# LemonATsu/DANBO-pytorch

Hardware: AMD Instinct MI355X
Metric: ray-samples/sec at 512x512x64 samples (higher is better)
Workload: dtype f32 (fp16x2-split MFMA products, fp32 accumulate); 1 GPU; H36M danbo_base network, 512x512 rays x (48 coarse + 16 importance) samples, 1 pose / 1 camera per rank, cylinder near/far, exact in-volume culling; rays=262144, samples_per_ray=64, parallelism=rays-dp1

## Files before the change

### danbo-pytorch_amd/core/_hip.py

```python
import ctypes
import os
import re
from ctypes import c_char_p, c_float, c_int, c_void_p
from types import SimpleNamespace

import torch

_HERE = os.path.dirname(os.path.abspath(__file__))
LIB_PATH = os.environ.get("DANBO_HIP_LIB") or os.path.join(os.path.dirname(_HERE), "libdanbo_hip.so")

P = c_void_p
I = c_int
F = c_float


class HeaderError(ValueError):
    """include/danbo_hip.h left the subset of C that parse_header reads"""


_SCALARS = {"int": c_int, "long": ctypes.c_long, "long long": ctypes.c_longlong, "size_t": ctypes.c_size_t, "float": c_float,
            **{f"{u}int{n}_t": getattr(ctypes, f"c_{u}int{n}") for u in ("", "u") for n in (8, 16, 32, 64)}}
_TAIL = r"((?:\*\s*(?:const\b\s*)?)*)(\w+)\s*(?:\[\s*(\w*)\s*\])?$"
_DECL = re.compile(r"(?:const\s+)?(long\s+long|\w+)\b\s*" + _TAIL)
_MORE = re.compile(_TAIL)
# ... 137 lines not shown
    return functions, structs, constants


def _header_path():
    env = os.environ.get("DANBO_HIP_HEADER")
    tried = [env] if env else [os.path.join(os.path.dirname(LIB_PATH), "danbo_hip.h"),
                               os.path.join(os.path.dirname(os.path.dirname(_HERE)), "include", "danbo_hip.h")]
    for p in tried:
        if os.path.exists(p):
            return p
    raise RuntimeError("danbo_hip.h not found (the ctypes binding is derived from it): tried " + ", ".join(tried)
                       + "; set DANBO_HIP_HEADER or put the header beside the library")


HEADER_PATH = _header_path()
with open(HEADER_PATH) as _f:
    _functions, _structs, _constants = parse_header(_f.read())
SIGNATURES = {name: argtypes for name, (_, argtypes) in _functions.items()}
RESTYPES = {name: restype for name, (restype, _) in _functions.items()}
STRUCTS = {name: type(name, (ctypes.Structure,), {"_fields_": fields, "__doc__": f"struct {name} of include/danbo_hip.h"})
           for name, fields in _structs.items()}
globals().update(STRUCTS)
C = SimpleNamespace(**_constants)
MAX_ROW_SPANS = C.DANBO_MAX_ROW_SPANS
ANERF_MAX_D = C.DANBO_ANERF_MAX_D

TRAIN_TENSORS = (
    ["graph_net.layers.0.lin.weight", "graph_net.layers.0.adj_w", "graph_net.layers.0.bias", "graph_net.layers.1.lin.weight",
     "graph_net.layers.1.adj_w", "graph_net.layers.1.bias", "graph_net.layers.2.weight", "graph_net.layers.2.bias",
     "graph_net.layers.3.weight", "graph_net.layers.3.bias", "graph_net.axis_scale",
     "prob_linears.layers.0.lin.weight", "prob_linears.layers.0.adj_w", "prob_linears.layers.0.bias", "prob_linears.layers.1.weight",
     "prob_linears.layers.1.bias", "prob_linears.layers.2.weight", "prob_linears.layers.2.bias"]
    + [f"pts_linears.{i}.weight" for i in range(8)] + [f"pts_linears.{i}.bias" for i in range(8)]
    + ["alpha_linear.weight", "alpha_linear.bias", "feature_linear.weight", "feature_linear.bias", "views_linears.0.weight",
       "views_linears.0.bias", "rgb_linear.weight", "rgb_linear.bias", "framecodes.codes.weight"])
N_TRAIN_TENSORS = C.DANBO_T_COUNT
_anchors = {"graph_net.axis_scale": C.DANBO_T_AXIS_SCALE, "prob_linears.layers.0.lin.weight": C.DANBO_T_A_W0,
            "pts_linears.0.weight": C.DANBO_T_PTS_W0, "pts_linears.0.bias": C.DANBO_T_PTS_B0, "alpha_linear.weight": C.DANBO_T_ALPHA_W,
            "framecodes.codes.weight": C.DANBO_T_CODES}
if len(TRAIN_TENSORS) != N_TRAIN_TENSORS or any(TRAIN_TENSORS.index(k) != i for k, i in _anchors.items()):
    raise HeaderError(f"TRAIN_TENSORS does not line up with enum DanboTrainTensor of {HEADER_PATH}")

_lib = None


def lib():
    global _lib
    if _lib is None:
        if not os.path.exists(LIB_PATH):
            raise RuntimeError(
                f"{LIB_PATH} not found: build it with `make -C danbo-pytorch_amd/csrc` "
                "(or __graft_entry__.build()).  There is no CPU / PyTorch fallback.")
        l = ctypes.CDLL(LIB_PATH)
        for name, argtypes in SIGNATURES.items():
            fn = getattr(l, name)
            fn.argtypes = argtypes
            fn.restype = RESTYPES[name]
        if l.danbo_abi_version() != C.DANBO_ABI_VERSION:
            raise RuntimeError(f"{LIB_PATH} has ABI version {l.danbo_abi_version()}, {HEADER_PATH} declares {C.DANBO_ABI_VERSION}: "
                               "the library is stale, rebuild it with `make -C danbo-pytorch_amd/csrc`")
        _lib = l
    return _lib


def ptr(t):
    return None if t is None else c_void_p(t.data_ptr())


def stream():
    return c_void_p(torch.cuda.current_stream().cuda_stream)


class HipError(RuntimeError):
    pass


def check(code, name):
    if code != 0:
        raise HipError(f"{name} failed with code {code}" + (" (invalid argument)" if code == C.DANBO_EINVAL else ""))

# ... 4 lines not shown
```

### danbo-pytorch_amd/core/hip_ops.py

```python
import ctypes

import torch

from . import _hip
from ._hip import call as _call, ptr as _p, stream as _stream

J = _hip.C.DANBO_J
VOL = _hip.C.DANBO_VOL
FEAT = _hip.C.DANBO_FEAT
RAY_FLAT_VMAX = _hip.C.DANBO_RAY_FLAT_VMAX
H_STRIDE = _hip.C.DANBO_H_STRIDE
MLP_PACKED_FLOATS = _hip.C.DANBO_MLP_PACKED_FLOATS
ASSIGN16_PACKED_BYTES = _hip.C.DANBO_ASSIGN16_PACKED_BYTES
MLP16_PACKED_BYTES = _hip.C.DANBO_MLP16_PACKED_BYTES
ANERF_ENC_FLOATS = _hip.C.DANBO_ANERF_ENC_FLOATS
LINEAR16_ENC_K = _hip.C.DANBO_LINEAR16_ENC_K
TRUNK_PACKED_BYTES = _hip.C.DANBO_TRUNK_PACKED_BYTES
TRUNK_PE_WIDTH = _hip.C.DANBO_TRUNK_PE_WIDTH
VIEW_W = 128


def _f32(t, name):
    if t is None:
        return None
# ... 70 lines not shown
        self.S = self.z.shape[1] if self.z is not None else self.pts.shape[1]
        self.M = self.R * self.S
        self.device = self.rays_o.device
        self.ray_mask = ray_mask if self.z is not None else None

    def head(self):
        return (_p(self.rays_o), _p(self.rays_d), _p(self.z), _p(self.pts), self.R, self.S, self.G,
                _p(self.skts), _p(self.align), _p(self.axis_scale))


def bone_cull(geo, compact=True, cnt=None):
    bits = torch.empty(geo.M, device=geo.device, dtype=torch.int32)
    lst = None
    if compact:
        lst = torch.empty(geo.M, device=geo.device, dtype=torch.int32)
        if cnt is None:
            cnt = torch.zeros(1, device=geo.device, dtype=torch.int32)
        assert cnt.dtype == torch.int32 and cnt.numel() == 1 and cnt.is_contiguous()
    else:
        cnt = None
    rm = tuple(geo.ray_mask) if geo.ray_mask is not None else (None, None, None)
    flat = rm[3] if len(rm) > 3 else None
    _call("danbo_bone_cull", *geo.head(), _p(rm[0]), _p(rm[1]), _p(rm[2]), _p(flat), _p(bits), _p(lst), _p(cnt), _stream())
    return bits, lst, cnt


def ray_bone_mask(rays_o, rays_d, skts, align, axis_scale, t_lo, t_hi, want_flat=False):
    rays_o, rays_d, skts = _f32(rays_o, "rays_o"), _f32(rays_d, "rays_d"), _f32(skts, "skts")
    t_lo, t_hi = _f32(t_lo, "t_lo").reshape(-1), _f32(t_hi, "t_hi").reshape(-1)
    R, G = rays_o.shape[0], skts.shape[0]
    assert t_lo.shape[0] == R and t_hi.shape[0] == R
    mask = torch.empty(R, device=rays_o.device, dtype=torch.int32)
    flat = torch.empty(R, device=rays_o.device, dtype=torch.int32) if want_flat else None
    _call("danbo_ray_bone_mask", _p(rays_o), _p(rays_d), _p(t_lo), _p(t_hi), R, G, _p(skts), _p(_f32(align, "align")),
          _p(_f32(axis_scale, "axis_scale")), _p(mask), _p(flat), _stream())
    return (mask, t_lo, t_hi, flat) if want_flat else (mask, t_lo, t_hi)


def group_rows(bits, lst, cnt):
    _call("danbo_group_rows", _p(bits), _p(lst), _p(cnt), lst.shape[0], _stream())
    return lst


def bone_gather(geo, volumes, lst=None, cnt=None, n=None):
    n = geo.M if n is None else n
    out = torch.empty(n, J, FEAT, device=geo.device, dtype=torch.float32)
# ... 618 lines not shown
```

### danbo-pytorch_amd/core/render_engine.py

```python
import ctypes

import torch

from . import _hip
from . import hip_ops as ops


class RenderEngine:
    fuse_resample = False

    def _key(self):
        return tuple((k, v.data_ptr(), v._version) for k, v in sorted(self.p.items()))

    def _sampling(self, N_samples, N_importance):
        cfg = self.cfg
        return (N_samples or cfg["N_samples"], N_importance or cfg["N_importance"], cfg["density_scale"],
                ops.density_act(cfg.get("density_act")))

    @staticmethod
    def frame_result(out, out0):
        return dict(rgb_map=out["rgb_map"], disp_map=out["disp_map"], acc_map=out["acc_map"], alpha=out["alpha"],
                    T_i=out["weights"], rgb0=out0["rgb_map"], disp0=out0["disp_map"], acc0=out0["acc_map"],
                    alpha0=out0["alpha"])

# ... 20 lines not shown
        ret = self.frame_result(out, out0)
        if keep:
            ret.update(near=near, far=far, z_coarse=z, raw_coarse=raw, weights_coarse=out0["weights"], z_fine=z_fine,
                       z_sorted=z_all, sorted_idxs=order, raw_fine=raw_f, **ex, **ex_f)
        return ret


class DanboEngine(RenderEngine):
    fuse_resample = True

    def __init__(self, cfg, params, align, buffers=None, mlp_mode="f16split"):
        self.cfg = cfg
        self.p = params
        self.align = align.float().contiguous()
        self._packed_key = None
        self.packed = self.wrt = self.empty_consts = None
        self.mean_code = None
        self.profile = None
        self.skip_flat_rays = True
        self.mlp_form = 32
        assert mlp_mode in ("f16split", "fp32")
        self.mlp_mode = mlp_mode
        self.group_rows = False

    def refresh(self):
        key = self._key()
        if key == self._packed_key and getattr(self, "_built_mode", None) == (self.mlp_mode, self.mlp_form):
            return
        p = self.p
        dev = p["alpha_linear.weight"].device
        q = self._equalized(p) if self.mlp_mode == "f16split" else p
        self.pts_w = [q[f"pts_linears.{i}.weight"] for i in range(8)]
        self.pts_b = [q[f"pts_linears.{i}.bias"].contiguous() for i in range(8)]
        self.packed, self.wrt = ops.mlp_pack(self.pts_w, q["feature_linear.weight"], q["views_linears.0.weight"])
        self.packed16, self.views_b16 = ops.mlp16_pack(self.pts_w, q["feature_linear.weight"],
                                                       q["feature_linear.bias"], q["views_linears.0.weight"],
                                                       q["views_linears.0.bias"], form=self.mlp_form)
        self.alpha_w = q["alpha_linear.weight"].reshape(-1).contiguous()
        self.alpha_b = q["alpha_linear.bias"].contiguous()
        self.feature_b = q["feature_linear.bias"].contiguous()
        self.views_b = q["views_linears.0.bias"].contiguous()
        self.rgb_w = q["rgb_linear.weight"].contiguous()
        self.rgb_b = q["rgb_linear.bias"].contiguous()
        self.view_scale = q.get("_view_scale", torch.ones((), device=dev))
        g = "graph_net.layers."
        self.gw = dict(
# ... 87 lines not shown
    def _mlp(self, h, S, cview, raw, lst=None, cnt=None, n=None, aux=False):
        if self.mlp_mode == "f16split":
            return ops.pe_mlp16(h, S, self.packed16, self.pts_b, self.alpha_w, self.alpha_b, cview,
                                self.rgb_w, self.rgb_b, raw, lst, cnt, n, aux, form=self.mlp_form)
        return ops.pe_mlp(h, S, self.packed, self.pts_b, self.alpha_w, self.alpha_b, self.feature_b, cview,
                          self.rgb_w, self.rgb_b, raw, lst, cnt, n, aux)

    def volumes(self, bones):
        self.refresh()
        return ops.pose_volumes(bones, self.gw, self.cfg["multires_graph"])

    def view_constants(self, rays_d, skts, cam_idx, ray_list=None, ray_count=None):
        self.refresh()
        cfg = self.cfg
        ray_mode = {"world": 0, "root_local": 1}[cfg["ray_tr_type"]]
        normalise = 1 if cfg["view_type"] == "relray" else 0
        return ops.view_consts(rays_d, skts, ray_mode, normalise, cfg["multires_views"], self.framecodes,
                               self.mean_code, cam_idx, self.wrt,
                               self.views_b16 if self.mlp_mode == "f16split" else self.views_b, self.rgb_w,
                               self.rgb_b, self.empty_consts, {16: 1, 32: 2}[self.mlp_form] if self.mlp_mode == "f16split" else 0,
                               self.code_table, ray_list, ray_count)

    def forward_samples(self, rays_o, rays_d, skts, bones, cam_idx=None, z=None, pts=None, dense=False,
                        want_confd=False, volumes=None, view=None, fill=True, ray_mask=None, count=None):
        self.refresh()
        geo = ops.Geometry(rays_o, rays_d, skts, self.align, self.axis_scale, z=z, pts=pts, ray_mask=ray_mask)
        vols = self.volumes(bones) if volumes is None else volumes
        cview, raw_empty = self.view_constants(geo.rays_d, geo.skts, cam_idx) if view is None else view
        S = geo.S
        bits, lst, cnt = ops.bone_cull(geo, compact=not dense, cnt=count)
        if lst is not None and self.mlp_mode == "f16split" and self.group_rows:
            ops.group_rows(bits, lst, cnt)
        if self.mlp_mode == "f16split":
            h, confd = ops.gather_assign_blend16(geo, vols, bits, self.aw, self.assign16, lst, cnt, geo.M, want_confd)
        else:
            h, confd = ops.gather_assign_blend(geo, vols, bits, self.aw, lst, cnt, geo.M, want_confd)
        raw = ops.fill_raw(raw_empty, S) if fill or dense else torch.empty(geo.R, S, 4, device=raw_empty.device)
        if self.profile is not None:
            e0, e1 = torch.cuda.Event(enable_timing=True), torch.cuda.Event(enable_timing=True)
            e0.record()
        self._mlp(h, S, cview, raw, lst, cnt, geo.M)
        if self.profile is not None:
            e1.record()
            self.profile.setdefault("k_pe_mlp", []).append((e0, e1, cnt if cnt is not None else geo.M))
        extras = dict(valid_bits=bits, list=lst, count=cnt, confd_rows=confd, h_rows=h, volumes=vols)
        return raw, extras

    def density(self, pts, skts, bones, netchunk=1024 * 64):
        self.refresh()
        M = pts.shape[0]
        out = torch.empty(M, 1, device=pts.device, dtype=torch.float32)
        vols = self.volumes(bones)
        for a in range(0, M, netchunk):
# ... 50 lines not shown
        m.density_scale, m.use_volume_near_far = float(cfg["density_scale"]), int(bool(cfg["use_volume_near_far"]))
        m.flat_rays_ok = int(self.flat_rays_ok and self.skip_flat_rays)
        r = _hip.DanboRays(rays_o=rays_o.data_ptr(), rays_d=rays_d.data_ptr(), skts=skts.data_ptr(), bones=bones.data_ptr(),
                           cyls=cyls.data_ptr(), cam_idx=None if cam is None else cam.data_ptr(), near_in=None, far_in=None,
                           R=R, G=G, chunk=int(chunk))
        shapes = dict(rgb_map=(R, 3), disp_map=(R,), acc_map=(R,), alpha=(R, S + Sf), weights=(R, S + Sf), rgb0=(R, 3),
                      disp0=(R,), acc0=(R,), alpha0=(R, S))
        out = {k: torch.empty(v, device=dev, dtype=torch.float32) for k, v in shapes.items()}
        o = _hip.DanboFrameOut(**{k: v.data_ptr() for k, v in out.items()})
        nbytes = _hip.lib().danbo_render_frame_workspace(R, G, S, Sf, int(chunk), m.graph_width)
        ws = torch.empty(nbytes, device=dev, dtype=torch.uint8)
        ops._call("danbo_render_frame_act", ctypes.byref(m), ctypes.byref(r), S, Sf, ctypes.byref(o), _hip.ptr(ws), nbytes,
                  *ops._act_args(act), ops._stream())
        out["T_i"] = out.pop("weights")
        return out

    def near_far(self, rays_o, rays_d, cyls, skts, near0=0.0, far0=1.0, chunk=4096):
        self.refresh()
        near, far = ops.near_far_cylinder(rays_o, rays_d, cyls, near0, far0, chunk)
        if self.cfg["use_volume_near_far"]:
            ops.near_far_boxes(rays_o, rays_d, skts, self.align, self.axis_scale, near, far)
        return near, far

    def render(self, rays_o, rays_d, skts, bones, cyls, cam_idx=None, N_samples=None, N_importance=None,
               chunk=4096, near_far=None, dense=False, keep=False):
        S, Sf, B, act = self._sampling(N_samples, N_importance)
        self.refresh()
        fused = S <= 64 and Sf <= 64
        lazy = not dense and not keep
        flat_mode = (lazy and (fused or (S <= 256 and Sf <= 64)) and self.skip_flat_rays and self.flat_rays_ok
                     and act[0] == "relu")
        near, far = self.near_far(rays_o, rays_d, cyls, skts, 0.0, 1.0, chunk) if near_far is None else near_far
        z = ops.coarse_samples(near, far, S)
        ray_mask = None if dense else ops.ray_bone_mask(rays_o, rays_d, skts, self.align, self.axis_scale, near, far,
                                                        want_flat=flat_mode)
        counts = torch.zeros(3, device=rays_o.device, dtype=torch.int32)
        flat = None
        vols = self.volumes(bones)
        if flat_mode:
            flat = ops.flat_rays(ray_mask[1], ray_mask[3], S, Sf, want_weights=not fused, cnt=counts[2:3])
            view = self.view_constants(rays_d, skts, cam_idx, flat["ray_list"], flat["ray_count"])
        else:
            view = self.view_constants(rays_d, skts, cam_idx)
        if ray_mask is not None:
            ray_mask = ray_mask[:3]
        raw, ex = self.forward_samples(rays_o, rays_d, skts, bones, cam_idx, z=z, dense=dense, volumes=vols, view=view,
                                       fill=not lazy, ray_mask=ray_mask, count=counts[0:1])
        if fused:
            out0, z_all, z_fine, order = ops.composite_importance(
                raw, z, rays_d, Sf, B, bits=ex["valid_bits"] if lazy else None, raw_empty=view[1] if lazy else None,
                want_weights=keep, flat=flat, act=act)
        else:
            out0 = ops.composite(raw, z, rays_d, B, bits=ex["valid_bits"] if lazy else None, raw_empty=view[1] if lazy else None,
                                 flat=flat, act=act)
            z_all, z_fine, order = ops.importance_samples(z, out0["weights"], Sf, flat=flat)
        raw_f, ex_f = self.forward_samples(rays_o, rays_d, skts, bones, cam_idx, z=z_fine, dense=dense,
                                           volumes=vols, view=view, fill=not lazy,
                                           ray_mask=ray_mask, count=counts[1:2])
        out = ops.composite_merged(raw, raw_f, order, z_all, rays_d, B, bits_a=ex["valid_bits"] if lazy else None,
                                   bits_b=ex_f["valid_bits"] if lazy else None, raw_empty=view[1] if lazy else None,
                                   want_raw=keep, flat=flat, act=act)
        ret = self.frame_result(out, out0)
        if keep:
            ret.update(near=near, far=far, z_coarse=z, raw_coarse=raw, weights_coarse=out0["weights"], z_fine=z_fine,
                       z_sorted=z_all, sorted_idxs=order, raw_fine=raw_f, raw_sorted=out.get("raw_sorted"),
                       count_coarse=ex["count"], count_fine=ex_f["count"], valid_bits=ex["valid_bits"])
        return ret

    def _network_pass(self, rays_o, rays_d, skts, bones, cam_idx, z, bounds, dense, lazy, tag):
        mask = None if dense else ops.ray_bone_mask(rays_o, rays_d, skts, self.align, self.axis_scale, *bounds)
        view = self.view_constants(rays_d, skts, cam_idx)
        raw, ex = self.forward_samples(rays_o, rays_d, skts, bones, cam_idx, z=z, dense=dense, volumes=self.volumes(bones), view=view,
                                       fill=not lazy, ray_mask=mask)
        bits, empty = (ex["valid_bits"], view[1]) if lazy else (None, None)
        return raw, bits, empty, {"count_" + tag: ex["count"], "valid_bits" + ("_fine" if tag == "fine" else ""): ex["valid_bits"]}
```

### danbo-pytorch_amd/csrc/common.hpp

```cpp
#pragma once
#include <hip/hip_runtime.h>
#include <stdint.h>
#include <algorithm>
#include <atomic>
#include "../../include/danbo_hip.h"
#include "sample_math.hpp"

#define DANBO_CHECK_ARG(cond) do { if (!(cond)) return DANBO_EINVAL; } while (0)
#define DANBO_CHECK_DENSITY_ACT(act, shift) \
    DANBO_CHECK_ARG(((act) == DANBO_DENSITY_RELU || (act) == DANBO_DENSITY_SOFTPLUS) && (shift) - (shift) == 0.f)
#define DANBO_LAUNCH_RET() do { hipError_t e_ = hipGetLastError(); return e_ == hipSuccess ? 0 : (int)e_; } while (0)

#define DANBO_ENSURE_LDS(func, bytes)                                                                              \
    do {                                                                                                           \
        static std::atomic<unsigned long long> done_{0};                                                           \
        int dev_ = 0;                                                                                              \
        if (hipGetDevice(&dev_) != hipSuccess) return (int)hipGetLastError();                                      \
        const unsigned long long bit_ = 1ull << (dev_ & 63);                                                       \
        if (!(done_.load(std::memory_order_acquire) & bit_)) {                                                     \
            const hipError_t e_ = hipFuncSetAttribute(reinterpret_cast<const void*>(func),                         \
                                                      hipFuncAttributeMaxDynamicSharedMemorySize, (int)(bytes));   \
            if (e_ != hipSuccess) return (int)e_;                                                                  \
            done_.fetch_or(bit_, std::memory_order_release);                                                       \
        }                                                                                                          \
    } while (0)

#if defined(__HIP_DEVICE_COMPILE__)
#define DANBO_NO_PK_F32 __attribute__((target("no-packed-fp32-ops")))
// ... 160 lines not shown
```

### danbo-pytorch_amd/csrc/k_frame.hip

```cpp
#include "common.hpp"

using namespace danbo;

namespace {
struct Carver {
    char* base;
    size_t used, cap;
    template <class T>
    T* take(size_t n) {
        used = (used + 255) & ~(size_t)255;
        T* p = base ? reinterpret_cast<T*>(base + used) : nullptr;
        used += n * sizeof(T);
        return p;
    }
};

struct FrameBuffers {
    float *near, *far, *cyl_scratch, *z, *vol_scratch, *volumes, *cview, *raw_empty, *h, *raw_a, *raw_b, *z_fine, *z_sorted, *weights0;
    uint32_t *bits_a, *bits_b, *ray_mask, *ray_flat;
    int32_t *list, *count, *order, *ray_list;
};

FrameBuffers carve(Carver& c, int R, int G, int S, int Sf, int chunk, int Wg) {
    FrameBuffers b;
// ... 31 lines not shown
    carve(c, R, G, S, Sf, chunk, graph_width);
    return c.used + 256;
}

#define DANBO_TRY(call) do { const int rc_ = (call); if (rc_ != 0) return rc_; } while (0)

static int render_frame_impl(const DanboModel* m, const DanboRays* r, int S, int Sf, const DanboFrameOut* o, void* workspace,
                             size_t workspace_bytes, int act, float shift, void* stream) {
    DANBO_CHECK_ARG(m && r && o && workspace && S >= 3 && S <= 256 && Sf >= 1 && Sf <= 64);
    DANBO_CHECK_ARG(r->R >= 1 && r->G >= 1 && r->R % r->G == 0 && r->chunk >= 1);
    DANBO_CHECK_ARG(r->rays_o && r->rays_d && r->skts && r->bones && r->cyls);
    DANBO_CHECK_ARG(o->rgb_map && o->disp_map && o->acc_map && o->alpha && o->weights && o->rgb0 && o->disp0 && o->acc0 && o->alpha0);
    const int R = r->R, G = r->G;
    const bool flat_rays = m->flat_rays_ok != 0 && act == DANBO_DENSITY_RELU;
    DANBO_CHECK_ARG(workspace_bytes >= danbo_render_frame_workspace(R, G, S, Sf, r->chunk, m->graph_width));
    Carver c{reinterpret_cast<char*>(((uintptr_t)workspace + 255) & ~(uintptr_t)255), 0, workspace_bytes};
    const FrameBuffers b = carve(c, R, G, S, Sf, r->chunk, m->graph_width);
    hipStream_t st = (hipStream_t)stream;

    DANBO_TRY(danbo_near_far_cylinder(r->rays_o, r->rays_d, r->cyls, R, G, 0.f, 1.f, r->near_in, r->far_in, r->chunk, b.cyl_scratch,
                                      b.near, b.far, stream));
    if (m->use_volume_near_far)
        DANBO_TRY(danbo_near_far_boxes(r->rays_o, r->rays_d, r->skts, m->align, m->axis_scale, R, G, b.near, b.far, stream));
    DANBO_TRY(danbo_coarse_samples(b.near, b.far, R, S, nullptr, b.z, stream));
    DANBO_TRY(danbo_ray_bone_mask(r->rays_o, r->rays_d, b.near, b.far, R, G, r->skts, m->align, m->axis_scale, b.ray_mask,
                                  flat_rays ? b.ray_flat : nullptr, stream));
    DANBO_TRY(danbo_pose_volumes_fwd(r->bones, G, m->L_graph, m->graph_width, m->g_w0, m->g_adjw0, m->g_b0, m->g_w1, m->g_adjw1, m->g_b1,
                                     m->g_w2, m->g_b2, m->g_w3, m->g_b3, b.vol_scratch, b.volumes, stream));
    zero_words(b.count, 4, nullptr, 0, st);
    auto view_consts = [&](const int32_t* ray_list, const int32_t* ray_count) -> int {
        return danbo_view_consts(r->rays_d, r->skts, R, G, m->ray_mode, m->normalise, m->L_view, m->framecodes, m->n_codes, m->code_size,
                                 m->mean_code, r->cam_idx, m->views_w_ray_t, m->views_b_eff, m->rgb_w, m->rgb_b, m->empty_consts, 2,
                                 m->code_table, ray_list, ray_count, b.cview, b.raw_empty, stream);
    };
    const int32_t *ray_list = nullptr, *ray_count = nullptr;
    if (flat_rays) {
        DANBO_TRY(danbo_flat_rays(b.near, b.ray_flat, R, S, Sf, o->rgb0, o->disp0, o->acc0, b.weights0, o->alpha0, b.z_fine, o->rgb_map,
                                  o->disp_map, o->acc_map, o->weights, o->alpha, b.ray_list, b.count + 3, 3, stream));
        ray_list = b.ray_list;
        ray_count = b.count + 3;
    }
    DANBO_TRY(view_consts(ray_list, ray_count));
    auto cull = [&](const float* zz, int s, uint32_t* bits, int32_t* count) -> int {
        DANBO_TRY(danbo_bone_cull(r->rays_o, r->rays_d, zz, nullptr, R, s, G, r->skts, m->align, m->axis_scale, b.ray_mask, b.near, b.far,
                                  nullptr, bits, b.list, count, stream));
        return 0;
    };
    auto network = [&](const float* zz, int s, uint32_t* bits, int32_t* count, float* raw) -> int {
        DANBO_TRY(danbo_gather_assign_blend16_fwd(r->rays_o, r->rays_d, zz, nullptr, R, s, G, r->skts, m->align, m->axis_scale, b.volumes,
                                                  bits, b.list, count, R * s, m->assign16, m->a_b0, m->a_b1, m->a_w2, m->a_b2, b.h,
                                                  nullptr, reinterpret_cast<uint32_t*>(b.count + 2), stream));
        return danbo_pe_mlp32_fwd(b.h, b.list, count, R * s, s, m->mlp16, m->pts_b, m->alpha_w, m->alpha_b, b.cview, m->rgb_w,
                                  m->rgb_b, raw, nullptr, stream);
    };
    DANBO_TRY(cull(b.z, S, b.bits_a, b.count));
    DANBO_TRY(network(b.z, S, b.bits_a, b.count, b.raw_a));
    if (S <= 64) {
        DANBO_TRY(danbo_composite_importance_pdf_fwd_act(b.raw_a, b.raw_empty, b.bits_a, b.z, r->rays_d, R, S, Sf, m->density_scale, nullptr,
                                                         nullptr, 0, o->rgb0, o->disp0, o->acc0, nullptr, o->alpha0, b.z_fine, b.z_sorted,
                                                         b.order, ray_list, ray_count, act, shift, stream));
    } else {
        DANBO_TRY(danbo_composite_rays_fwd_act(b.raw_a, b.raw_empty, b.bits_a, b.z, r->rays_d, R, S, m->density_scale, nullptr, o->rgb0,
                                               o->disp0, o->acc0, b.weights0, o->alpha0, ray_list, ray_count, act, shift, stream));
        DANBO_TRY(danbo_importance_samples_rays(b.z, b.weights0, R, S, Sf, nullptr, b.z_fine, b.z_sorted, b.order, ray_list, ray_count,
                                                stream));
    }
// ... 18 lines not shown
```

### danbo-pytorch_amd/csrc/k_sample.hip

```cpp
#include "common.hpp"

namespace danbo {

__global__ __launch_bounds__(256) DANBO_NO_PK_F32 void k_cylinder_pass1(const float* __restrict__ rays_o,
                                                        const float* __restrict__ rays_d,
                                                        const float* __restrict__ cyl, int R, int G,
                                                        float near0, float far0,
                                                        const float* __restrict__ near_in,
                                                        const float* __restrict__ far_in, int chunk,
                                                        double* __restrict__ acc,
                                                        float* __restrict__ near_out,
                                                        float* __restrict__ far_out) {
    const int rays_per_pose = R / G;
    for (int r0 = blockIdx.x * blockDim.x; r0 < R; r0 += gridDim.x * blockDim.x) {
        const int r = r0 + threadIdx.x;
        const bool act = r < R;
        const int rc = act ? r : R - 1;
        const int g = min(rc / rays_per_pose, G - 1);
        float o[3] = {rays_o[3 * rc], rays_o[3 * rc + 1], rays_o[3 * rc + 2]};
        float d[3] = {rays_d[3 * rc], rays_d[3 * rc + 1], rays_d[3 * rc + 2]};
        float c[3] = {cyl[5 * g], cyl[5 * g + 1], cyl[5 * g + 2]};
        float nr, fr;
        const bool hit = cylinder_bounds(o, d, c, near_in ? near_in[rc] : near0, far_in ? far_in[rc] : far0, &nr, &fr) && act;
        if (act) {
// ... 490 lines not shown
    if (list != nullptr) {
        __shared__ int s_cnt[CULL_SPT * (CULL_BLOCK / 64)];
        __shared__ int s_base;
        const int wave = threadIdx.x >> 6;
        unsigned long long ball[CULL_SPT];
#pragma unroll
        for (int it = 0; it < CULL_SPT; ++it) {
            ball[it] = __ballot(bits4[it] != 0);
            if (lane == 0) s_cnt[it * (CULL_BLOCK / 64) + wave] = __popcll(ball[it]);
        }
        __syncthreads();
        if (threadIdx.x == 0) {
            int run = 0;
            for (int i = 0; i < CULL_SPT * (CULL_BLOCK / 64); ++i) { const int c = s_cnt[i]; s_cnt[i] = run; run += c; }
            s_base = run > 0 ? atomicAdd(count, run) : 0;
        }
        __syncthreads();
#pragma unroll
        for (int it = 0; it < CULL_SPT; ++it) {
            if (bits4[it] != 0) {
                const long m = base + it * CULL_BLOCK + threadIdx.x;
                list[s_base + s_cnt[it * (CULL_BLOCK / 64) + wave] + __popcll(ball[it] & ((1ull << lane) - 1ull))] = (int32_t)m;
            }
        }
    }
}

constexpr int GATHER_TS = 16;
constexpr int GATHER_BLOCK = GATHER_TS * J;

__global__ __launch_bounds__(GATHER_BLOCK) void k_bone_gather(const float* __restrict__ rays_o,
                                                              const float* __restrict__ rays_d,
                                                              const float* __restrict__ z,
                                                              const float* __restrict__ pts, int R, int S, int G,
                                                              const float* __restrict__ skts,
                                                              const float* __restrict__ align,
                                                              const float* __restrict__ axis_scale,
                                                              const float* __restrict__ volumes,
                                                              const int32_t* __restrict__ list,
                                                              const int32_t* __restrict__ count, int n_cap,
                                                              float* __restrict__ part_feat) {
    __shared__ __attribute__((aligned(16))) float s_vol[J * VOL];
    __shared__ __attribute__((aligned(16))) float s_out[GATHER_TS * J * FEAT];
    __shared__ __attribute__((aligned(16))) float s_skt[J * 16];
    __shared__ __attribute__((aligned(16))) float s_align[J * 16];
    __shared__ float s_scale[J * 4];
// ... 607 lines not shown

extern "C" int danbo_bone_cull(const float* rays_o, const float* rays_d, const float* z, const float* pts, int R, int S, int G,
                                const float* skts, const float* align, const float* axis_scale, const uint32_t* ray_mask,
                                const float* t_lo, const float* t_hi, uint32_t* ray_flat, uint32_t* valid_bits, int32_t* list,
                                int32_t* count, void* stream) {
    DANBO_CHECK_ARG(R > 0 && S > 0 && G > 0 && R % G == 0);
    DANBO_CHECK_ARG((list == nullptr) == (count == nullptr));
    DANBO_CHECK_ARG((z == nullptr) != (pts == nullptr));
    DANBO_CHECK_ARG(ray_mask == nullptr || (z != nullptr && t_lo != nullptr && t_hi != nullptr));
    DANBO_CHECK_ARG(ray_flat == nullptr || ray_mask != nullptr);
    const long M = (long)R * S;
    const long spp = (long)(R / G) * S;
    const int per_block = CULL_BLOCK * CULL_SPT;
    long np = per_block / spp + 2;
    if (np > G) np = G;
    const size_t lds = sizeof(float) * (J * 16 + J * 4 + np * J * 16);
    DANBO_CHECK_ARG(lds <= 64 * 1024);
    const int grid = ceil_div(M, per_block);
    hipLaunchKernelGGL(k_bone_cull, dim3(grid), dim3(CULL_BLOCK), lds, (hipStream_t)stream, rays_o, rays_d, z, pts, R, S,
                       G, skts, align, axis_scale, (int)np, ray_mask, t_lo, t_hi, ray_flat, valid_bits, list, count);
    DANBO_LAUNCH_RET();
}

extern "C" int danbo_ray_bone_mask(const float* rays_o, const float* rays_d, const float* t_lo, const float* t_hi, int R, int G,
                                    const float* skts, const float* align, const float* axis_scale, uint32_t* ray_mask,
                                    uint32_t* ray_flat, void* stream) {
    DANBO_CHECK_ARG(rays_o && rays_d && t_lo && t_hi && skts && align && axis_scale && ray_mask);
    DANBO_CHECK_ARG(R > 0 && G > 0 && R % G == 0);
    const long np = 256 / (R / G) + 2 < G ? 256 / (R / G) + 2 : G;
    const bool in_lds = np <= 8;
    const size_t lds = sizeof(float) * (J * 16 + J * 4 + (in_lds ? np * J * 16 : 0));
    if (in_lds)
        hipLaunchKernelGGL(k_ray_bone_mask<true>, dim3(ceil_div(R, 256)), dim3(256), lds, (hipStream_t)stream, rays_o, rays_d, t_lo, t_hi,
                           skts, align, axis_scale, R, G, ray_mask, ray_flat);
    else
        hipLaunchKernelGGL(k_ray_bone_mask<false>, dim3(ceil_div(R, 256)), dim3(256), lds, (hipStream_t)stream, rays_o, rays_d, t_lo,
                           t_hi, skts, align, axis_scale, R, G, ray_mask, ray_flat);
    DANBO_LAUNCH_RET();
}

extern "C" int danbo_bone_gather_fwd(const float* rays_o, const float* rays_d, const float* z, const float* pts, int R, int S, int G,
                                      const float* skts, const float* align, const float* axis_scale,
                                      const float* volumes, const int32_t* list, const int32_t* count, int n,
                                      float* part_feat, void* stream) {
    DANBO_CHECK_ARG(R > 0 && S > 0 && G > 0 && R % G == 0 && n >= 0);
    DANBO_CHECK_ARG((z == nullptr) != (pts == nullptr));
// ... 227 lines not shown
```

Measured before the change: 4.146 billion ray-samples/s.

## Cull samples only over listed non-flat rays, fusing coarse depth generation

Adds a bone-cull kernel that walks the compacted ray list from flat_rays instead of every sample of every ray. Each block takes a window of listed rays, computes coarse depths on the fly and writes them out, which replaces the separate coarse_samples pass. It then tests bone volumes and compacts the surviving sample rows with an LDS histogram that can optionally group rows by bone pair. Rays left out of the list never get coarse depths or valid bits written, so downstream code must not read them. The per-block ray grouping also adds LDS scan overhead.

```diff
diff --git a/danbo-pytorch_amd/core/_hip.py b/danbo-pytorch_amd/core/_hip.py
--- a/danbo-pytorch_amd/core/_hip.py
+++ b/danbo-pytorch_amd/core/_hip.py
@@ -183,6 +183,20 @@
            for name, fields in _structs.items()}
 globals().update(STRUCTS)
 C = SimpleNamespace(**_constants)
+COMPANION_HEADERS = ("danbo_hip_rays.h",)
+COMPANION_SIGNATURES, COMPANION_RESTYPES, _companion_constants = {}, {}, {}
+for _name in COMPANION_HEADERS:
+    _path = os.path.join(os.path.dirname(HEADER_PATH), _name)
+    if not os.path.exists(_path):
+        raise RuntimeError(f"{_path} not found: it belongs beside {HEADER_PATH}")
+    with open(_path) as _f:
+        _fns, _sts, _cons = parse_header(_f.read())
+    if _sts or set(_fns) & (set(SIGNATURES) | set(COMPANION_SIGNATURES)) or set(_cons) & (set(_constants) | set(_companion_constants)):
+        raise HeaderError(f"{_path}: a companion header declares entry points and constants only, each once")
+    _companion_constants.update(_cons)
+    COMPANION_SIGNATURES.update({name: argtypes for name, (_, argtypes) in _fns.items()})
+    COMPANION_RESTYPES.update({name: restype for name, (restype, _) in _fns.items()})
+COMPANION_C = SimpleNamespace(**_companion_constants)
 MAX_ROW_SPANS = C.DANBO_MAX_ROW_SPANS
 ANERF_MAX_D = C.DANBO_ANERF_MAX_D
 
@@ -213,10 +227,10 @@
                 f"{LIB_PATH} not found: build it with `make -C danbo-pytorch_amd/csrc` "
                 "(or __graft_entry__.build()).  There is no CPU / PyTorch fallback.")
         l = ctypes.CDLL(LIB_PATH)
-        for name, argtypes in SIGNATURES.items():
+        for name, argtypes in {**SIGNATURES, **COMPANION_SIGNATURES}.items():
             fn = getattr(l, name)
             fn.argtypes = argtypes
-            fn.restype = RESTYPES[name]
+            fn.restype = RESTYPES[name] if name in RESTYPES else COMPANION_RESTYPES[name]
         if l.danbo_abi_version() != C.DANBO_ABI_VERSION:
             raise RuntimeError(f"{LIB_PATH} has ABI version {l.danbo_abi_version()}, {HEADER_PATH} declares {C.DANBO_ABI_VERSION}: "
                                "the library is stale, rebuild it with `make -C danbo-pytorch_amd/csrc`")
diff --git a/danbo-pytorch_amd/core/hip_ops.py b/danbo-pytorch_amd/core/hip_ops.py
--- a/danbo-pytorch_amd/core/hip_ops.py
+++ b/danbo-pytorch_amd/core/hip_ops.py
@@ -116,6 +116,46 @@
     rm = tuple(geo.ray_mask) if geo.ray_mask is not None else (None, None, None)
     flat = rm[3] if len(rm) > 3 else None
     _call("danbo_bone_cull", *geo.head(), _p(rm[0]), _p(rm[1]), _p(rm[2]), _p(flat), _p(bits), _p(lst), _p(cnt), _stream())
+    return bits, lst, cnt
+
+
+CULL_RAYS_MAX_WINDOW = _hip.COMPANION_C.DANBO_CULL_RAYS_MAX_WINDOW
+CULL_RAYS_MAX_RPW = _hip.COMPANION_C.DANBO_CULL_RAYS_MAX_RPW
+
+
+def cull_rays_check(R, S, ray_mask, ray_list, ray_count, near_far=None, rpw=0):
+    if ray_mask is None or len(ray_mask) < 3 or any(t is None for t in ray_mask[:3]):
+        raise ValueError("bone_cull_rays needs ray_bone_mask()'s (mask, t_lo, t_hi) of the rays")
+    if any(t.numel() != R for t in ray_mask[:3]) or ray_mask[0].dtype != torch.int32:
+        raise ValueError("ray mask, t_lo, t_hi: one entry per ray, the mask int32")
+    if ray_list is None or ray_count is None:
+        raise ValueError("bone_cull_rays walks a ray list: pass flat_rays()'s ray_list and ray_count (no list: bone_cull)")
+    if ray_list.dtype != torch.int32 or ray_list.numel() < R or not ray_list.is_contiguous():
+        raise ValueError("ray_list: contiguous int32 with room for every ray")
+    if ray_count.dtype != torch.int32 or ray_count.numel() != 1:
+        raise ValueError("ray_count: one int32")
+    if near_far is not None and any(t.dtype != torch.float32 or t.numel() != R or not t.is_contiguous() for t in near_far):
+        raise ValueError("near_far: two contiguous float32 [R]")
+    rpw = int(rpw)
+    if rpw < 0 or rpw > CULL_RAYS_MAX_RPW or max(rpw, 1) * S > CULL_RAYS_MAX_WINDOW:
+        raise ValueError(f"rays per window {rpw} x {S} samples: at most {CULL_RAYS_MAX_RPW} rays and {CULL_RAYS_MAX_WINDOW} samples")
+    return rpw
+
+
+def bone_cull_rays(geo, ray_list, ray_count, cnt=None, near_far=None, by_bone=True, rpw=0):
+    if geo.z is None:
+        raise ValueError("bone_cull_rays works on depths along rays (Geometry(z=...)), not on points")
+    rpw = cull_rays_check(geo.R, geo.S, geo.ray_mask, ray_list, ray_count, near_far, rpw)
+    bits = torch.empty(geo.M, device=geo.device, dtype=torch.int32)
+    lst = torch.empty(geo.M, device=geo.device, dtype=torch.int32)
+    if cnt is None:
+        cnt = torch.zeros(1, device=geo.device, dtype=torch.int32)
+    assert cnt.dtype == torch.int32 and cnt.numel() == 1 and cnt.is_contiguous()
+    rm = geo.ray_mask
+    nf = (None, None) if near_far is None else near_far
+    _call("danbo_bone_cull_rays", _p(geo.rays_o), _p(geo.rays_d), _p(None if near_far is not None else geo.z), _p(nf[0]), _p(nf[1]),
+          _p(geo.z if near_far is not None else None), geo.R, geo.S, geo.G, _p(geo.skts), _p(geo.align), _p(geo.axis_scale),
+          _p(rm[0]), _p(rm[1]), _p(rm[2]), _p(ray_list), _p(ray_count), rpw, int(bool(by_bone)), _p(bits), _p(lst), _p(cnt), _stream())
     return bits, lst, cnt
 
 
diff --git a/danbo-pytorch_amd/core/render_engine.py b/danbo-pytorch_amd/core/render_engine.py
--- a/danbo-pytorch_amd/core/render_engine.py
+++ b/danbo-pytorch_amd/core/render_engine.py
@@ -66,6 +66,8 @@
         assert mlp_mode in ("f16split", "fp32")
         self.mlp_mode = mlp_mode
         self.group_rows = False
+        self.cull_listed_rays = True
+        self.cull_rows_by_bone = False
 
     def refresh(self):
         key = self._key()
@@ -199,13 +201,17 @@
                                self.code_table, ray_list, ray_count)
 
     def forward_samples(self, rays_o, rays_d, skts, bones, cam_idx=None, z=None, pts=None, dense=False,
-                        want_confd=False, volumes=None, view=None, fill=True, ray_mask=None, count=None):
+                        want_confd=False, volumes=None, view=None, fill=True, ray_mask=None, count=None, rays=None, near_far=None):
         self.refresh()
         geo = ops.Geometry(rays_o, rays_d, skts, self.align, self.axis_scale, z=z, pts=pts, ray_mask=ray_mask)
         vols = self.volumes(bones) if volumes is None else volumes
         cview, raw_empty = self.view_constants(geo.rays_d, geo.skts, cam_idx) if view is None else view
         S = geo.S
-        bits, lst, cnt = ops.bone_cull(geo, compact=not dense, cnt=count)
+        if rays is not None:
+            assert not dense
+            bits, lst, cnt = ops.bone_cull_rays(geo, rays[0], rays[1], cnt=count, near_far=near_far, by_bone=self.cull_rows_by_bone)
+        else:
+            bits, lst, cnt = ops.bone_cull(geo, compact=not dense, cnt=count)
         if lst is not None and self.mlp_mode == "f16split" and self.group_rows:
             ops.group_rows(bits, lst, cnt)
         if self.mlp_mode == "f16split":
@@ -302,6 +308,9 @@
             ops.near_far_boxes(rays_o, rays_d, skts, self.align, self.axis_scale, near, far)
         return near, far
 
+    def list_cull(self, flat_mode):
+        return bool(flat_mode) and bool(self.cull_listed_rays)
+
     def render(self, rays_o, rays_d, skts, bones, cyls, cam_idx=None, N_samples=None, N_importance=None,
                chunk=4096, near_far=None, dense=False, keep=False):
         S, Sf, B, act = self._sampling(N_samples, N_importance)
@@ -311,21 +320,24 @@
         flat_mode = (lazy and (fused or (S <= 256 and Sf <= 64)) and self.skip_flat_rays and self.flat_rays_ok
                      and act[0] == "relu")
         near, far = self.near_far(rays_o, rays_d, cyls, skts, 0.0, 1.0, chunk) if near_far is None else near_far
-        z = ops.coarse_samples(near, far, S)
         ray_mask = None if dense else ops.ray_bone_mask(rays_o, rays_d, skts, self.align, self.axis_scale, near, far,
                                                         want_flat=flat_mode)
         counts = torch.zeros(3, device=rays_o.device, dtype=torch.int32)
         flat = None
         vols = self.volumes(bones)
+        rays = None
         if flat_mode:
             flat = ops.flat_rays(ray_mask[1], ray_mask[3], S, Sf, want_weights=not fused, cnt=counts[2:3])
+            rays = (flat["ray_list"], flat["ray_count"]) if self.list_cull(flat_mode) else None
             view = self.view_constants(rays_d, skts, cam_idx, flat["ray_list"], flat["ray_count"])
         else:
             view = self.view_constants(rays_d, skts, cam_idx)
         if ray_mask is not None:
             ray_mask = ray_mask[:3]
+        z = ops.coarse_samples(near, far, S) if rays is None else torch.empty(ray_mask[1].shape[0], S, device=rays_o.device)
         raw, ex = self.forward_samples(rays_o, rays_d, skts, bones, cam_idx, z=z, dense=dense, volumes=vols, view=view,
-                                       fill=not lazy, ray_mask=ray_mask, count=counts[0:1])
+                                       fill=not lazy, ray_mask=ray_mask, count=counts[0:1], rays=rays,
+                                       near_far=None if rays is None else (ray_mask[1], ray_mask[2]))
         if fused:
             out0, z_all, z_fine, order = ops.composite_importance(
                 raw, z, rays_d, Sf, B, bits=ex["valid_bits"] if lazy else None, raw_empty=view[1] if lazy else None,
@@ -336,7 +348,7 @@
             z_all, z_fine, order = ops.importance_samples(z, out0["weights"], Sf, flat=flat)
         raw_f, ex_f = self.forward_samples(rays_o, rays_d, skts, bones, cam_idx, z=z_fine, dense=dense,
                                            volumes=vols, view=view, fill=not lazy,
-                                           ray_mask=ray_mask, count=counts[1:2])
+                                           ray_mask=ray_mask, count=counts[1:2], rays=rays)
         out = ops.composite_merged(raw, raw_f, order, z_all, rays_d, B, bits_a=ex["valid_bits"] if lazy else None,
                                    bits_b=ex_f["valid_bits"] if lazy else None, raw_empty=view[1] if lazy else None,
                                    want_raw=keep, flat=flat, act=act)
diff --git a/danbo-pytorch_amd/csrc/common.hpp b/danbo-pytorch_amd/csrc/common.hpp
--- a/danbo-pytorch_amd/csrc/common.hpp
+++ b/danbo-pytorch_amd/csrc/common.hpp
@@ -4,6 +4,7 @@
 #include <algorithm>
 #include <atomic>
 #include "../../include/danbo_hip.h"
+#include "../../include/danbo_hip_rays.h"
 #include "sample_math.hpp"
 
 #define DANBO_CHECK_ARG(cond) do { if (!(cond)) return DANBO_EINVAL; } while (0)
diff --git a/danbo-pytorch_amd/csrc/k_frame.hip b/danbo-pytorch_amd/csrc/k_frame.hip
--- a/danbo-pytorch_amd/csrc/k_frame.hip
+++ b/danbo-pytorch_amd/csrc/k_frame.hip
@@ -77,7 +77,7 @@
                                       b.near, b.far, stream));
     if (m->use_volume_near_far)
         DANBO_TRY(danbo_near_far_boxes(r->rays_o, r->rays_d, r->skts, m->align, m->axis_scale, R, G, b.near, b.far, stream));
-    DANBO_TRY(danbo_coarse_samples(b.near, b.far, R, S, nullptr, b.z, stream));
+    if (!flat_rays) DANBO_TRY(danbo_coarse_samples(b.near, b.far, R, S, nullptr, b.z, stream));
     DANBO_TRY(danbo_ray_bone_mask(r->rays_o, r->rays_d, b.near, b.far, R, G, r->skts, m->align, m->axis_scale, b.ray_mask,
                                   flat_rays ? b.ray_flat : nullptr, stream));
     DANBO_TRY(danbo_pose_volumes_fwd(r->bones, G, m->L_graph, m->graph_width, m->g_w0, m->g_adjw0, m->g_b0, m->g_w1, m->g_adjw1, m->g_b1,
@@ -97,6 +97,9 @@
     }
     DANBO_TRY(view_consts(ray_list, ray_count));
     auto cull = [&](const float* zz, int s, uint32_t* bits, int32_t* count) -> int {
+        if (ray_list != nullptr)
+            return danbo_bone_cull_rays(r->rays_o, r->rays_d, zz == b.z ? nullptr : zz, b.near, b.far, b.z, R, s, G, r->skts, m->align,
+                                        m->axis_scale, b.ray_mask, b.near, b.far, ray_list, ray_count, 0, 0, bits, b.list, count, stream);
         DANBO_TRY(danbo_bone_cull(r->rays_o, r->rays_d, zz, nullptr, R, s, G, r->skts, m->align, m->axis_scale, b.ray_mask, b.near, b.far,
                                   nullptr, bits, b.list, count, stream));
         return 0;
diff --git a/danbo-pytorch_amd/csrc/k_sample.hip b/danbo-pytorch_amd/csrc/k_sample.hip
--- a/danbo-pytorch_amd/csrc/k_sample.hip
+++ b/danbo-pytorch_amd/csrc/k_sample.hip
@@ -536,6 +536,207 @@
                 const long m = base + it * CULL_BLOCK + threadIdx.x;
                 list[s_base + s_cnt[it * (CULL_BLOCK / 64) + wave] + __popcll(ball[it] & ((1ull << lane) - 1ull))] = (int32_t)m;
             }
+        }
+    }
+}
+
+constexpr int CULLR_BLOCK = 256;
+constexpr int CULLR_MAX_TURNS = 16;
+constexpr int CULLR_MAX_RAYS = 256;
+constexpr int CULLR_KEYS = 25 * 25;
+constexpr int CULLR_NO_ROW = 0xffff;
+static_assert(CULLR_BLOCK * CULLR_MAX_TURNS == DANBO_CULL_RAYS_MAX_WINDOW && CULLR_MAX_RAYS == DANBO_CULL_RAYS_MAX_RPW,
+              "danbo_hip_rays.h states the window limits");
+
+__global__ __launch_bounds__(CULLR_BLOCK) void k_bone_cull_rays(const float* __restrict__ rays_o, const float* __restrict__ rays_d,
+                                                                const float* __restrict__ z, const float* __restrict__ near,
+                                                                const float* __restrict__ far, float* __restrict__ z_out,
+                                                                int R, int S, int G, const float* __restrict__ skts,
+                                                                const float* __restrict__ align, const float* __restrict__ axis_scale,
+                                                                const uint32_t* __restrict__ ray_mask, const float* __restrict__ t_lo,
+                                                                const float* __restrict__ t_hi, const int32_t* __restrict__ ray_list,
+                                                                const int32_t* __restrict__ ray_count, int rpw, int turns, int by_bone,
+                                                                uint32_t* __restrict__ valid_bits, int32_t* __restrict__ list,
+                                                                int32_t* __restrict__ count) {
+    __shared__ __attribute__((aligned(16))) float s_align[J * 16];
+    __shared__ __attribute__((aligned(16))) float s_skt[J * 16];
+    __shared__ __attribute__((aligned(16))) float s_scale[J * 4];
+    __shared__ int s_ray[CULLR_MAX_RAYS];
+    __shared__ uint32_t s_rmask[CULLR_MAX_RAYS];
+    __shared__ float s_lo[CULLR_MAX_RAYS], s_hi[CULLR_MAX_RAYS], s_near[CULLR_MAX_RAYS], s_far[CULLR_MAX_RAYS];
+    __shared__ unsigned short s_key[CULLR_BLOCK * CULLR_MAX_TURNS];
+    __shared__ int s_hist[CULLR_BLOCK / 64][CULLR_KEYS];
+    __shared__ int s_wsum[CULLR_BLOCK / 64];
+    __shared__ int s_base;
+
+    const int n_listed = resolve_count(ray_count, R);
+    const int e0 = blockIdx.x * rpw;
+    if (e0 >= n_listed) return;
+    const int nr = min(rpw, n_listed - e0);
+    const int nwin = nr * S;
+    const int tid = threadIdx.x, lane = tid & 63, wave = tid >> 6;
+    const int rays_per_pose = R / G;
+    auto pose_of = [&](int r) { return G == 1 ? 0 : min(r / rays_per_pose, G - 1); };
+    const float inv_S = 1.0f / (float)S;
+    auto entry_of = [&](int li) {
+        int q = (int)((float)li * inv_S);
+        q -= (q * S > li) ? 1 : 0;
+        q += ((q + 1) * S <= li) ? 1 : 0;
+        return q;
+    };
+    if (tid < nr) {
+        const int r = min(max(ray_list[e0 + tid], 0), R - 1);
+        const float lo = t_lo[r], hi = t_hi[r];
+        const float slack = 5e-5f * fmaxf(fabsf(lo), fabsf(hi));
+        s_ray[tid] = r;
+        s_rmask[tid] = ray_mask[r];
+        s_lo[tid] = lo - slack;
+        s_hi[tid] = hi + slack;
+        if (z == nullptr) { s_near[tid] = near[r]; s_far[tid] = far[r]; }
+    }
+    for (int i = tid; i < (CULLR_BLOCK / 64) * CULLR_KEYS; i += CULLR_BLOCK) (&s_hist[0][0])[i] = 0;
+    for (int i = tid; i < J * 16; i += CULLR_BLOCK) s_align[i] = align[i];
+    for (int i = tid; i < J * 4; i += CULLR_BLOCK) s_scale[i] = (i & 3) < 3 ? fabsf(axis_scale[(i >> 2) * 3 + (i & 3)]) : 0.f;
+    __syncthreads();
+    const int g0 = pose_of(s_ray[0]);
+    for (int i = tid; i < J * 16; i += CULLR_BLOCK) s_skt[i] = skts[(size_t)g0 * J * 16 + i];
+    __syncthreads();
+
+    const int li0 = wave * turns * 64 + lane;
+    for (int pr = 0; pr < turns / 2; ++pr) {
+        const int lia = li0 + (2 * pr) * 64, lib = lia + 64;
+        const bool acta = lia < nwin, actb = lib < nwin;
+        if (!__builtin_amdgcn_readfirstlane((int)__any(acta))) {
+            s_key[lia] = CULLR_NO_ROW;
+            s_key[lib] = CULLR_NO_ROW;
+            continue;
+        }
+        const int lac = min(lia, nwin - 1), lbc = min(lib, nwin - 1);
+        const int ea = entry_of(lac), eb = entry_of(lbc);
+        const int sa = lac - ea * S, sb = lbc - eb * S;
+        const int ra = s_ray[ea], rb = s_ray[eb];
+        const long ma = (long)ra * S + sa, mb = (long)rb * S + sb;
+        const float oa[3] = {rays_o[3 * ra], rays_o[3 * ra + 1], rays_o[3 * ra + 2]};
+        const float da[3] = {rays_d[3 * ra], rays_d[3 * ra + 1], rays_d[3 * ra + 2]};
+        const float ob[3] = {rays_o[3 * rb], rays_o[3 * rb + 1], rays_o[3 * rb + 2]};
+        const float db[3] = {rays_d[3 * rb], rays_d[3 * rb + 1], rays_d[3 * rb + 2]};
+        float za, zb;
+        if (z != nullptr) {
+            za = z[ma];
+            zb = z[mb];
+        } else {
+            za = coarse_sample(s_near[ea], s_far[ea], sa, S, nullptr, ma);
+            zb = coarse_sample(s_near[eb], s_far[eb], sb, S, nullptr, mb);
+            if (acta) z_out[ma] = za;
+            if (actb) z_out[mb] = zb;
+        }
+        const uint32_t prea = !acta ? 0u : (za >= s_lo[ea] && za <= s_hi[ea]) ? s_rmask[ea] : (1u << J) - 1u;
+        const uint32_t preb = !actb ? 0u : (zb >= s_lo[eb] && zb <= s_hi[eb]) ? s_rmask[eb] : (1u << J) - 1u;
+        uint32_t need = wave_or(prea | preb);
+        uint32_t ba = 0u, bb = 0u;
+        if (need) {
+            float pa[3], pb[3];
+            sample_point(oa, da, za, pa);
+            sample_point(ob, db, zb, pb);
+            const int ga = pose_of(ra), gb = pose_of(rb);
+            if (__builtin_amdgcn_readfirstlane((int)__all(ga == g0 && gb == g0))) {
+                const v2f px = {pa[0], pb[0]}, py = {pa[1], pb[1]}, pz = {pa[2], pb[2]};
+                while (need) {
+                    const int j = __builtin_ctz(need);
+                    need &= need - 1u;
+                    v2f l[3], t[3];
+                    affine_pk(s_skt + 16 * j, px, py, pz, l);
+                    affine_pk(s_align + 16 * j, l[0], l[1], l[2], t);
+                    const float* sc = s_scale + 4 * j;
+                    const bool ina = !(fabsf(t[0].x) > sc[0] || fabsf(t[1].x) > sc[1] || fabsf(t[2].x) > sc[2]);
+                    const bool inb = !(fabsf(t[0].y) > sc[0] || fabsf(t[1].y) > sc[1] || fabsf(t[2].y) > sc[2]);
+                    ba |= (ina ? 1u : 0u) << j;
+                    bb |= (inb ? 1u : 0u) << j;
+                }
+            } else {
+                const float* ska = skts + (size_t)ga * J * 16;
+                const float* skb = skts + (size_t)gb * J * 16;
+                for (int j = 0; j < J; ++j) {
+                    float pt[3];
+                    bone_local(ska + 16 * j, s_align + 16 * j, pa, pt);
+                    ba |= (in_volume(pt, s_scale + 4 * j) ? 1u : 0u) << j;
+                    bone_local(skb + 16 * j, s_align + 16 * j, pb, pt);
+                    bb |= (in_volume(pt, s_scale + 4 * j) ? 1u : 0u) << j;
+                }
+            }
+        }
+        if (!acta) ba = 0u;
+        if (!actb) bb = 0u;
+        if (acta) valid_bits[ma] = ba;
+        if (actb) valid_bits[mb] = bb;
+        auto key_of = [&](uint32_t b) {
+            if (b == 0u) return CULLR_NO_ROW;
+            if (!by_bone) return 0;
+            const uint32_t rest = b & (b - 1u);
+            return __builtin_ctz(b) * 25 + (rest ? __builtin_ctz(rest) : 24);
+        };
+        const int ka = key_of(ba), kb = key_of(bb);
+        s_key[lia] = (unsigned short)ka;
+        s_key[lib] = (unsigned short)kb;
+        if (ka != CULLR_NO_ROW) atomicAdd(&s_hist[wave][ka], 1);
+        if (kb != CULLR_NO_ROW) atomicAdd(&s_hist[wave][kb], 1);
+    }
+    if (list == nullptr) return;
+    __syncthreads();
+    {
+        int c[3][CULLR_BLOCK / 64];
+        int mine = 0;
+#pragma unroll
+        for (int q = 0; q < 3; ++q)
+#pragma unroll
+            for (int w = 0; w < CULLR_BLOCK / 64; ++w) {
+                const int k = 3 * tid + q;
+                c[q][w] = k < CULLR_KEYS ? s_hist[w][k] : 0;
+                mine += c[q][w];
+            }
+        int inc = mine;
+        for (int d = 1; d < 64; d <<= 1) {
+            const int v = __shfl_up(inc, d);
+            if (lane >= d) inc += v;
+        }
+        if (lane == 63) s_wsum[wave] = inc;
+        __syncthreads();
+        int run = inc - mine, total = 0;
+#pragma unroll
+        for (int w = 0; w < CULLR_BLOCK / 64; ++w) {
+            run += w < wave ? s_wsum[w] : 0;
+            total += s_wsum[w];
+        }
+        if (tid == 0) s_base = total > 0 ? atomicAdd(count, total) : 0;
+#pragma unroll
+        for (int q = 0; q < 3; ++q)
+#pragma unroll
+            for (int w = 0; w < CULLR_BLOCK / 64; ++w) {
+                const int k = 3 * tid + q;
+                if (k < CULLR_KEYS) s_hist[w][k] = run;
+                run += c[q][w];
+            }
+        __syncthreads();
+    }
+    volatile int* cursor = &s_hist[wave][0];
+    const int row0 = s_base;
+    for (int t = 0; t < turns; ++t) {
+        const int li = li0 + t * 64;
+        const int key = s_key[li];
+        const bool row = key != CULLR_NO_ROW;
+        unsigned long long rem = __ballot(row);
+        int pos = 0;
+        while (rem != 0ull) {
+            const int k0 = __builtin_amdgcn_readlane(key, (int)__builtin_ctzll(rem));
+            const unsigned long long same = __ballot(row && key == k0);
+            const int first = cursor[k0];
+            if (row && key == k0) pos = first + (int)__popcll(same & ((1ull << lane) - 1ull));
+            if (lane == 0) cursor[k0] = first + (int)__popcll(same);
+            rem &= ~same;
+        }
+        if (row) {
+            const int e = entry_of(li);
+            list[row0 + pos] = (int32_t)((long)s_ray[e] * S + (li - e * S));
         }
     }
 }
@@ -1189,6 +1390,30 @@
     DANBO_LAUNCH_RET();
 }
 
+extern "C" int danbo_bone_cull_rays_rpw(int S) {
+    if (S < 1 || S > CULLR_BLOCK * CULLR_MAX_TURNS) return 0;
+    const int rpw = (S >= 32 ? 3072 : 2048) / S;
+    return rpw < 1 ? 1 : rpw > CULLR_MAX_RAYS ? CULLR_MAX_RAYS : rpw;
+}
+
+extern "C" int danbo_bone_cull_rays(const float* rays_o, const float* rays_d, const float* z, const float* near, const float* far,
+                                     float* z_out, int R, int S, int G, const float* skts, const float* align,
+                                     const float* axis_scale, const uint32_t* ray_mask, const float* t_lo, const float* t_hi,
+                                     const int32_t* ray_list, const int32_t* ray_count, int rpw, int by_bone, uint32_t* valid_bits,
+                                     int32_t* list, int32_t* count, void* stream) {
+    DANBO_CHECK_ARG(R > 0 && S > 0 && G > 0 && R % G == 0 && (long)R * S <= 0x7fffffffL);
+    DANBO_CHECK_ARG(rays_o && rays_d && skts && align && axis_scale && ray_mask && t_lo && t_hi && ray_list && ray_count && valid_bits);
+    DANBO_CHECK_ARG((list == nullptr) == (count == nullptr));
+    DANBO_CHECK_ARG(z != nullptr || (near != nullptr && far != nullptr && z_out != nullptr));
+    if (rpw == 0) rpw = danbo_bone_cull_rays_rpw(S);
+    DANBO_CHECK_ARG(rpw >= 1 && rpw <= CULLR_MAX_RAYS && (long)rpw * S <= CULLR_BLOCK * CULLR_MAX_TURNS);
+    const int turns = 2 * ceil_div((long)rpw * S, 2 * CULLR_BLOCK);
+    hipLaunchKernelGGL(k_bone_cull_rays, dim3(ceil_div(R, rpw)), dim3(CULLR_BLOCK), 0, (hipStream_t)stream, rays_o, rays_d, z, near,
+                       far, z_out, R, S, G, skts, align, axis_scale, ray_mask, t_lo, t_hi, ray_list, ray_count, rpw, turns,
+                       by_bone != 0 ? 1 : 0, valid_bits, list, count);
+    DANBO_LAUNCH_RET();
+}
+
 extern "C" int danbo_ray_bone_mask(const float* rays_o, const float* rays_d, const float* t_lo, const float* t_hi, int R, int G,
                                     const float* skts, const float* align, const float* axis_scale, uint32_t* ray_mask,
                                     uint32_t* ray_flat, void* stream) {
diff --git a/include/danbo_hip_rays.h b/include/danbo_hip_rays.h
--- /dev/null
+++ b/include/danbo_hip_rays.h
@@ -0,0 +1,26 @@
+#ifndef DANBO_HIP_RAYS_H
+#define DANBO_HIP_RAYS_H
+
+#include <stdint.h>
+
+#ifdef __cplusplus
+extern "C" {
+#endif
+
+#define DANBO_CULL_RAYS_MAX_WINDOW 4096
+#define DANBO_CULL_RAYS_MAX_RPW 256
+
+int danbo_bone_cull_rays(const float* rays_o, const float* rays_d, const float* z ,
+                         const float* near , const float* far , float* z_out ,
+                         int R, int S, int G, const float* skts, const float* align, const float* axis_scale,
+                         const uint32_t* ray_mask , const float* t_lo , const float* t_hi ,
+                         const int32_t* ray_list , const int32_t* ray_count , int rpw, int by_bone,
+                         uint32_t* valid_bits , int32_t* list , int32_t* count ,
+                         void* stream);
+int danbo_bone_cull_rays_rpw(int S);
+
+#ifdef __cplusplus
+}
+#endif
+
+#endif
```

New measurement: 4.193 billion ray-samples/s (median of 6 runs). +1.1%, better.
